# HJakeCunningham/ASVGP

Hardware: AMD Instinct MI355X
Metric: Mpoints/s per ELBO+grad step, N=10M 1D Matern-3/2 M=2048 (higher is better)
Workload: dtype f64

## Files before the change

asvgp_amd/_lib.py:

```python
import ctypes
import os

import torch

HERE = os.path.dirname(os.path.abspath(__file__))
LIB_PATH = os.path.join(HERE, "libasvgp_hip.so")

_c = ctypes
_P, _I, _L, _D, _Z = _c.c_void_p, _c.c_int, _c.c_int64, _c.c_double, _c.c_size_t

SIGNATURES = {
    "asvgp_version": (_I, []),
    "asvgp_last_error_string": (_c.c_char_p, []),
    "asvgp_status_name": (_c.c_char_p, [_I]),
    "asvgp_phi_workspace_bytes": (_Z, [_L, _I, _L]),
    "asvgp_create": (_I, [_c.POINTER(_P)]),
    "asvgp_destroy": (_I, [_P]),
    "asvgp_phi_accumulate_1d": (_I, [_P, _P, _P, _L, _L, _P, _L, _D, _I, _L, _P, _P, _Z, _P]),
    "asvgp_phi_weighted_workspace_bytes": (_Z, [_L, _I, _L]),
    "asvgp_phi_accumulate_1d_weighted": (_I, [_P, _P, _P, _P, _L, _L, _P, _L, _D, _I, _L, _P, _P, _P, _Z, _P]),
    "asvgp_set_weight_sums": (_I, [_P, _D, _D, _D]),
    "asvgp_phi_accumulate_kron2d_weighted": (_I, [_P, _P, _P, _L, _P, _L, _D, _L, _P, _L, _D, _L, _I, _P, _P, _P]),
    "asvgp_phi_accumulate_kron2d_sorted_weighted": (_I, [_P, _P, _P, _L, _P, _P, _L, _D, _L, _P, _L, _D, _L, _I, _P, _P, _P]),
    "asvgp_set_phi_algorithm": (_I, [_P, _I]),
    "asvgp_phi_last_algorithm": (_I, [_P]),
    "asvgp_set_phi_input_order": (_I, [_P, _I]),
    "asvgp_phi_last_input_order": (_I, [_P]),
    "asvgp_stream_probe": (_I, [_P, _P, _L, _P, _P]),
    "asvgp_debug_reload_env": (_I, []),
    "asvgp_set_deferred_forward_pass": (_I, [_P, _I]),
    "asvgp_prior_publish": (_I, [_P]),
    "asvgp_host_mantissa_bits": (_I, []),
    "asvgp_prior_interior_kuu_host": (_I, [_P, _I, _L, _I, _P, _P, _c.POINTER(_L), _c.POINTER(_L), _P]),
    "asvgp_result_mirror": (_I, [_P, _I, _c.POINTER(_P)]),
    "asvgp_result_mirror_read": (_I, [_P, _c.c_uint64, _P, _D]),
    "asvgp_elbo_grad_ahead_1d": (_I, [_P, _P, _P, _I, _L, _L, _I, _L, _P, _P, _P, _Z, _P]),
    "asvgp_elbo_publish_theta": (_I, [_P, _D, _D, _D]),
    "asvgp_elbo_grad_host_1d": (_I, [_P, _P, _P, _I, _D, _D, _D, _L, _L, _I, _L, _P, _P, _P, _Z, _P, _P, _D]),
    "asvgp_result_mirror_pending": (_c.c_uint64, [_P]),
    "asvgp_set_phi_workgroups": (_I, [_P, _I]),
    "asvgp_set_phi_deferred_reduce": (_I, [_P, _I]),
    "asvgp_phi_reduce_1d": (_I, [_P, _P]),
    "asvgp_phi_index_1d": (_I, [_P, _L, _P, _L, _D, _P, _P]),
    "asvgp_phi_evaluate_1d": (_I, [_P, _L, _P, _L, _D, _I, _I, _P, _P, _P]),
    "asvgp_matern_coeffs": (_I, [_I, _D, _D, _c.POINTER(_D), _c.POINTER(_D), _c.POINTER(_I)]),
    "asvgp_kuu_assemble": (_I, [_P, _I, _c.POINTER(_D), _c.POINTER(_D), _L, _I, _P, _P, _P]),
    "asvgp_cholesky_band": (_I, [_P, _P, _L, _I, _P, _P]),
    "asvgp_inverse_from_cholesky_band": (_I, [_P, _P, _L, _I, _P]),
    "asvgp_solve_triang_mat": (_I, [_P, _P, _P, _L, _I, _L, _I, _P]),
    "asvgp_product_band_band": (_I, [_P, _P, _P, _L, _I, _I, _I, _I, _I, _I, _P]),
    "asvgp_transpose_band": (_I, [_P, _P, _L, _I, _I, _P]),
    "asvgp_symmetrise_band": (_I, [_P, _P, _L, _I, _P]),
    "asvgp_unpack_banded_matrix_to_dense": (_I, [_P, _P, _L, _I, _I, _P]),
    "asvgp_pack_dense_matrix_to_banded": (_I, [_P, _P, _L, _I, _I, _P]),
    "asvgp_band_trace_sym": (_I, [_P, _P, _L, _I, _P, _P]),
    "asvgp_cholesky_band_vjp": (_I, [_P, _P, _P, _P, _L, _I, _P]),
    "asvgp_inverse_from_cholesky_band_vjp": (_I, [_P, _P, _P, _P, _P, _L, _I, _P]),
    "asvgp_band_outer_product": (_I, [_P, _P, _L, _L, _I, _D, _P, _P]),
    "asvgp_elbo_workspace_bytes": (_Z, [_L, _I, _L]),
    "asvgp_set_band_algorithm": (_I, [_P, _I]),
    "asvgp_prior_plan_1d": (_I, [_P, _P, _I, _L, _I, _c.POINTER(_I)]),
    "asvgp_prior_table_doubles": (_Z, [_P, _I, _L, _I]),
    "asvgp_prior_forward_host": (_I, [_P, _I, _L, _I, _P, _P, _P, _Z, _P]),
    "asvgp_set_prior_forward": (_I, [_P, _I]),
# ... 144 lines not shown
            self._mirror = None
            return None
        self._mirror = np.ctypeslib.as_array(ctypes.cast(ptr, ctypes.POINTER(_D)), shape=(16,))
        return self._mirror

    def set_deferred_forward_pass(self, on):
        check(self._lib.asvgp_set_deferred_forward_pass(self.ptr, int(on)), "set_deferred_forward_pass")

    def publish_forward(self):
        self._lib.asvgp_prior_publish(self.ptr)

    def result_mirror_pending(self):
        return int(self._lib.asvgp_result_mirror_pending(self.ptr))

    def set_phi_workgroups(self, n):
        check(self._lib.asvgp_set_phi_workgroups(self.ptr, int(n)), "set_phi_workgroups")

    deferred = False

    def set_phi_deferred_reduce(self, on):
        check(self._lib.asvgp_set_phi_deferred_reduce(self.ptr, int(on)), "set_phi_deferred_reduce")
        self.deferred = bool(on)

    def chain_sync(self, on):
        check(self._lib.asvgp_elbo_chain_sync(self.ptr, int(on)), "elbo_chain_sync")

    def prior_plan(self, static_stack_host, n_terms, M, k):
        ok = _I(0)
        ptr = None if static_stack_host is None else static_stack_host.ctypes.data
        check(self._lib.asvgp_prior_plan_1d(self.ptr, ptr, int(n_terms), int(M), int(k), ctypes.byref(ok)), "prior_plan_1d")
        return bool(ok.value)

    def close(self):
        if getattr(self, "ptr", None) is not None and self.ptr:
            try:
                self._lib.asvgp_destroy(self.ptr)
            except Exception:
                pass
            self.ptr = None
            self._mirror = None

    def __del__(self):
        self.close()


def set_default_algorithms(band=None, phi=None, prior_forward=None, phi_order=None):
# ... 45 lines not shown
```

asvgp_amd/csrc/handle.hip:

```cpp
#include <sched.h>
#include <stdlib.h>
#include <string.h>
#include <time.h>

#include <condition_variable>
#include <mutex>
#include <thread>
#include <vector>

#include "handle.hpp"

namespace asvgp {

static DebugEnv g_dbg;
static std::once_flag g_dbg_once;
static void debug_env_load() {
  g_dbg.no_assembly = getenv("ASVGP_DEBUG_NO_ASSEMBLY") ? 1 : 0;
  g_dbg.chain_stamps = getenv("ASVGP_CHAIN_STAMPS") ? 1 : 0;
  g_dbg.spin_limit = getenv("ASVGP_SPIN_LIMIT") ? atol(getenv("ASVGP_SPIN_LIMIT")) : (1L << 25);
  g_dbg.host_times = getenv("ASVGP_HOST_TIMES") ? 1 : 0;
  g_dbg.plan_first = getenv("ASVGP_PLAN_FIRST") ? 1 : 0;
  g_dbg.bcr_stamps = getenv("ASVGP_BCR_STAMPS") ? atoi(getenv("ASVGP_BCR_STAMPS")) : 0;
  g_dbg.no_split = getenv("ASVGP_NO_SPLIT") ? atoi(getenv("ASVGP_NO_SPLIT")) : 0;
}
const DebugEnv& debug_env() {
  std::call_once(g_dbg_once, debug_env_load);
  return g_dbg;
}

static Handle* g_default = nullptr;
static std::mutex g_default_mu;

Handle* as_handle(asvgp_handle_t h) {
  if (h) return reinterpret_cast<Handle*>(h);
  std::lock_guard<std::mutex> lk(g_default_mu);
  if (!g_default) {
    g_default = new Handle;
    (void)hipGetDevice(&g_default->device);
  }
  return g_default;
}

static void handle_quiesce(Handle* h) {
  if (h->ahead.valid) (void)elbo_publish_theta(h, 1.0, 1.0, 1.0, true);
  handle_publish_forward(h);
  bool need_sync = false;
// ... 164 lines not shown
  return ASVGP_OK;
}

extern "C" int asvgp_create(asvgp_handle_t* out) {
  if (!out) { set_error("asvgp_create: bad argument"); return ASVGP_ERR_BAD_ARG; }
  Handle* h = new Handle;
  if (hipGetDevice(&h->device) != hipSuccess) { delete h; set_error("asvgp_create: no HIP device"); return ASVGP_ERR_HIP; }
  *out = reinterpret_cast<asvgp_handle_t>(h);
  return ASVGP_OK;
}

extern "C" int asvgp_destroy(asvgp_handle_t handle) {
  if (!handle) return ASVGP_OK;
  Handle* h = reinterpret_cast<Handle*>(handle);
  if (h->magic != 0x41535647u) { set_error("asvgp_destroy: not a handle"); return ASVGP_ERR_BAD_ARG; }
  worker_stop(h);
  plan_release(h);
  if (h->mirror_host) (void)hipHostFree(h->mirror_host);
  if (h->evK) (void)hipEventDestroy(h->evK);
  if (h->evP) (void)hipEventDestroy(h->evP);
  if (h->prof_made)
    for (int i = 0; i < PROF_RING; ++i) { (void)hipEventDestroy(h->prof_ev[i][0]); (void)hipEventDestroy(h->prof_ev[i][1]); }
  if (h->order_dev) { (void)hipFree(h->order_dev); h->order_dev = nullptr; }
  if (h->box_host) { (void)hipHostFree(h->box_host); h->box_host = nullptr; h->box_dev = nullptr; }
  h->magic = 0;
  delete h;
  return ASVGP_OK;
}

extern "C" int asvgp_set_phi_algorithm(asvgp_handle_t handle, int algo) {
  if (algo != 0 && algo != 1 && algo != 3 && algo != 5 && algo != 6) {
    set_error("set_phi_algorithm: 0 auto (6 where it applies, else 5, else 3), 1 fp64 LDS-atomic band scatter, 3 fixed-point band scatter, 5 fixed-point centred-moment scatter, 6 tile sort + register moments");
    return ASVGP_ERR_BAD_ARG;
  }
  as_handle(handle)->phi_algo = algo;
  return ASVGP_OK;
}

extern "C" int asvgp_set_phi_input_order(asvgp_handle_t handle, int order) {
  if (order < 0 || order > 2) { set_error("set_phi_input_order: 0 probe once per (x, N), 1 unsorted, 2 time series"); return ASVGP_ERR_BAD_ARG; }
  Handle* h = as_handle(handle);
  h->phi_order = order;
  h->n_order_seen = 0;
  return ASVGP_OK;
}

// ... 2 lines not shown
extern "C" int asvgp_set_phi_workgroups(asvgp_handle_t handle, int n) {
  if (n < 0 || n > 256) { set_error("set_phi_workgroups: 0 (default, one per CU) .. 256"); return ASVGP_ERR_BAD_ARG; }
  as_handle(handle)->phi_blocks = n;
  return ASVGP_OK;
}

extern "C" int asvgp_set_weight_sums(asvgp_handle_t handle, double n_pos, double sum_w, double sum_log_w) {
  Handle* h = as_handle(handle);
  if (n_pos < 0.0) { h->w_set = false; h->w_npos = h->w_sum = h->w_sumlog = 0.0; return ASVGP_OK; }
  if (!(n_pos == n_pos) || n_pos != (double)(long long)n_pos || n_pos > 9.0e15 || !(sum_w >= 0.0) || !(sum_w < 1e300) || !(fabs(sum_log_w) < 1e300)) {
    set_error("set_weight_sums: n_pos must be a whole number of rows (negative: unweighted), sum_w >= 0 and sum_log_w finite");
    return ASVGP_ERR_BAD_ARG;
  }
  h->w_set = true; h->w_npos = n_pos; h->w_sum = sum_w; h->w_sumlog = sum_log_w;
  return ASVGP_OK;
}

extern "C" int asvgp_set_phi_deferred_reduce(asvgp_handle_t handle, int on) {
  Handle* h = as_handle(handle);
  h->phi_defer = on != 0;
  if (!h->phi_defer) h->pend.valid = false;
  return ASVGP_OK;
}

extern "C" int asvgp_set_band_algorithm(asvgp_handle_t handle, int algo) {
  if (algo < 0 || algo > 4) {
    set_error("set_band_algorithm: 0 auto, 1 sequential sweeps, 2 block cyclic reduction on the GPU, 3 block cyclic reduction with the planned (host, long double) prior forward pass, 4 the planned chains on the matrix cores");
    return ASVGP_ERR_BAD_ARG;
  }
  as_handle(handle)->band_algo = algo;
  return ASVGP_OK;
}

extern "C" int asvgp_set_deferred_forward_pass(asvgp_handle_t handle, int on) {
  Handle* h = as_handle(handle);
  if (on < 0 || on > 2) { set_error("set_deferred_forward_pass: 0 inline, 1 the caller publishes (asvgp_prior_publish), 2 the handle's worker thread"); return ASVGP_ERR_BAD_ARG; }
  handle_publish_forward(h);
  if (on != 2) worker_stop(h);
  h->defer_forward = on == 1;
  h->fwd_worker = on == 2;
  return ASVGP_OK;
}

extern "C" int asvgp_prior_publish(asvgp_handle_t handle) {
  handle_publish_forward(as_handle(handle));
  return ASVGP_OK;
// ... 143 lines not shown
```

asvgp_amd/csrc/handle.hpp:

```cpp
#pragma once
#include "asvgp_common.hpp"
#include "prior_plan.hpp"

namespace asvgp {

constexpr int PROF_RING = 1024;
constexpr int TAB_SLOTS = 16;

struct Handle {
  unsigned magic = 0x41535647u;
  int device = 0;
  int phi_algo = 0, phi_blocks = 0;
  int phi_last = 0;
  bool phi_defer = false;
  struct PendingReduce { const double* partials; int G, M, K; double* stats; bool valid; const int* ranges; } pend = {nullptr, 0, 0, 0, nullptr, false, nullptr};
  int band_algo = 0;
  bool sync_on = false;
  hipEvent_t evK = nullptr, evP = nullptr;
  bool prof_on = false, prof_made = false;
  int prof_every = 1;
  long prof_calls = 0, prof_n = 0;
  hipEvent_t prof_ev[PROF_RING][2];
  PriorPlan* plan = nullptr;
  int* node_rec_dev = nullptr;
// ... 12 lines not shown
  void* worker_park = nullptr;
  int wstate = 0;
  struct PendingForward { bool valid; double coef[ASVGP_MAX_KUU_TERMS], dcoef[ASVGP_MAX_KUU_TERMS]; double* tab; int slot; unsigned long long seq; } fwd = {false, {0}, {0}, nullptr, 0, 0};
  bool prior_forward_gpu = false;
  int* dd_img_i = nullptr;
  int dd_n_img = 0;
  double* dd_img_d = nullptr;
  double* dd_tab = nullptr;
  hipStream_t dd_stream = nullptr;
  unsigned long long* dd_ready = nullptr;
  double* mirror_host = nullptr;
  double* mirror_dev = nullptr;
  unsigned long long mirror_seq = 0;
  unsigned long long mirror_pending = 0;
  struct MeshSeen { const double* ptr; long n; int regular; double step, first, last; };
  MeshSeen mesh_seen[8];
  int n_mesh_seen = 0;
  int phi_order = 0;
  struct OrderSeen { const double* ptr; long n; int series; };
  OrderSeen order_seen[8];
  int n_order_seen = 0;
  int* order_dev = nullptr;
  int phi_last_series = 0;
  bool ahead_req = false;
  void* box_host = nullptr;
  void* box_dev = nullptr;
  struct PendingAhead { bool valid; int slot; unsigned long long seq; double* tab; int kind; double N, Nw, cw; } ahead = {false, 0, 0, nullptr, 0, 0.0, 0.0, 0.0};
  bool w_set = false;
  double w_npos = 0.0, w_sum = 0.0, w_sumlog = 0.0;
};
constexpr size_t BOX_BYTES = 4096;

struct DebugEnv { int no_assembly; int chain_stamps; long spin_limit; int host_times; int plan_first; int bcr_stamps; int no_split; };
const DebugEnv& debug_env();

Handle* as_handle(asvgp_handle_t h);

bool handle_mesh_is_linspace(Handle* h, const double* mesh_dev, long n_mesh, hipStream_t st, double* step_out, double* first_out, double* last_out);

int handle_flush_phi_reduce(Handle* h, const double* stats, hipStream_t st);

void handle_publish_forward(Handle* h);
void handle_post_forward(Handle* h);

int handle_prior_dd_prepare(Handle* h);
void handle_prior_dd_release(Handle* h);
int handle_prior_dd_forward(Handle* h, const double* coef, const double* dcoef, int slot, hipStream_t st, double** tab_out, unsigned long long* stamps = nullptr,
                            unsigned long long seq = 0, const unsigned long long** ready_out = nullptr);

int elbo_publish_theta(Handle* h, double v, double l, double s, bool withdraw);

double* handle_table_acquire(Handle* h, unsigned long long* seq_out, int* slot_out);

}
```

asvgp_amd/csrc/phi_pass.hip:

```cpp
#include <stdlib.h>

#include "handle.hpp"

namespace asvgp {

constexpr int PHI_THREADS = 1024;
constexpr int PHI_CH = 32;
constexpr int PHI_MAX_BLOCKS = 256;
constexpr size_t PHI_LDS_BUDGET = 160 * 1024 - 512;

template <int K> struct FxTab {
  int g[K + 1];
  constexpr FxTab() : g{} {
    double cf[K + 1][K + 1] = {};
    for (int i = 0; i <= K; ++i)
      for (int p = 0; p <= K; ++p) cf[i][p] = piece_coef<K, 0>(i, p);
    for (int d = 0; d <= K; ++d) {
      double mx = 0.0;
      for (int i = 0; i + d <= K; ++i)
        for (int q = 0; q <= 32; ++q) {
          const double t = q / 32.0;
          double a = cf[i][K], b = cf[i + d][K];
          for (int p = K - 1; p >= 0; --p) { a = a * t + cf[i][p]; b = b * t + cf[i + d][p]; }
          if (a * b > mx) mx = a * b;
// ... 658 lines not shown
  if (lane == 0 && good) atomicAdd(count, 1);
}

static bool handle_phi_is_series(Handle* h, const double* x, long N, double m0, double inv_delta, long n_mesh, hipStream_t st) {
  if (h->phi_order == 1) return false;
  if (h->phi_order == 2) return true;
  for (int i = 0; i < h->n_order_seen; ++i)
    if (h->order_seen[i].ptr == x && h->order_seen[i].n == N) return h->order_seen[i].series != 0;
  int series = 0;
  const int nprobe = 512;
  if (N >= 128L * nprobe) {
    if (!h->order_dev && hipMalloc(&h->order_dev, sizeof(int)) != hipSuccess) h->order_dev = nullptr;
    int cnt = 0;
    if (h->order_dev && hipMemsetAsync(h->order_dev, 0, sizeof(int), st) == hipSuccess) {
      hipLaunchKernelGGL(phi_order_probe_kernel, dim3(nprobe), dim3(64), 0, st, x, N, N / nprobe, nprobe, m0, inv_delta, (int)n_mesh, h->order_dev);
      if (hipMemcpyAsync(&cnt, h->order_dev, sizeof(int), hipMemcpyDeviceToHost, st) == hipSuccess && hipStreamSynchronize(st) == hipSuccess)
        series = cnt * 10 >= nprobe * 9 ? 1 : 0;
    }
  }
  if (h->n_order_seen < 8) h->order_seen[h->n_order_seen++] = Handle::OrderSeen{x, N, series};
  return series != 0;
}

template <int K, int TP, int TS>
static int launch_phi_sort_as(Handle* h, const double* x, const double* y, long N, const double* mesh, long n_mesh, double delta,
                              long M, double* stats, double* ws, hipStream_t st, double step, double m0, double m_last, double margin) {
  size_t lds_bytes = ps_lds_bytes<K, TP, TS>();
  if (ps_epilogue_bytes<K>() > lds_bytes) lds_bytes = ps_epilogue_bytes<K>();
  if (lds_bytes > 160 * 1024) return 1;
  long nblk = (N + TP * PS_THREADS - 1) / (TP * PS_THREADS);
  const long gmax = (h->phi_blocks > 0 && h->phi_blocks < PHI_MAX_BLOCKS) ? h->phi_blocks : PHI_MAX_BLOCKS;
  const int G = (int)(nblk < 1 ? 1 : (nblk > gmax ? gmax : nblk));
  long ppb = (N + G - 1) / G;
  ppb = TS ? ((ppb + 127) & ~127L) : ((ppb + 1) & ~1L);
  if (ppb > 0x3fffffffL) return 1;
  PsArgs a;
  a.x = x; a.y = y; a.N = N; a.mesh_g = mesh; a.n_mesh = (int)n_mesh; a.inv_delta = 1.0 / delta; a.M = (int)M;
  a.m0 = m0; a.m_last = m_last; a.step = step; a.smax_fast = 0.5 - margin;
  a.partials = ws; a.ppb = ppb; a.zero_ptr = stats; a.zero_n = (K + 2) * M + 1; a.stamps = nullptr; a.stamps_wave = 0;
  a.ranges = reinterpret_cast<int*>(ws + (size_t)PHI_MAX_BLOCKS * ((size_t)(K + 2) * M + 1));
  auto kern = phi_sort_kernel<K, TP, 0, 1, TS>;
  hipError_t e = hipFuncSetAttribute(reinterpret_cast<const void*>(kern), hipFuncAttributeMaxDynamicSharedMemorySize, (int)lds_bytes);
  if (e != hipSuccess) { set_error("hipFuncSetAttribute(%zu B LDS): %s", lds_bytes, hipGetErrorString(e)); return ASVGP_ERR_LDS_CAPACITY; }
  const bool prof = h->prof_on && h->prof_n < PROF_RING && (h->prof_calls++ % h->prof_every == 0);
  if (prof) (void)hipEventRecord(h->prof_ev[h->prof_n][0], st);
  hipLaunchKernelGGL(kern, dim3((unsigned)G), dim3(PS_THREADS), lds_bytes, st, a);
  if (prof) { (void)hipEventRecord(h->prof_ev[h->prof_n][1], st); ++h->prof_n; }
  h->phi_last_series = TS;
  const int E1 = (int)((K + 2) * M + 1);
  const int gsplit = G >= 64 ? 16 : (G >= 8 ? 4 : 1);
  if (h->phi_defer) {
    h->pend = Handle::PendingReduce{a.partials, G, (int)M, K, stats, true, a.ranges};
    return check_launch("phi_accumulate_1d (tile sort, reduce deferred)");
  }
  hipLaunchKernelGGL(phi_reduce_kernel, dim3((E1 + 255) / 256, gsplit), dim3(256), 0, st, a.partials, G, (int)M, K, 0, M, 1L, 0, 1, stats, (const int*)a.ranges);
  return check_launch("phi_accumulate_1d (tile sort)");
}

template <int K>
static int launch_phi_sort(Handle* h, const double* x, const double* y, long N, long D, const double* mesh, long n_mesh, double delta,
                           long M, double* stats, double* ws, hipStream_t st) {
  if (D != 1 || N < 2 || M > PS_NCELL || ((reinterpret_cast<uintptr_t>(x) | reinterpret_cast<uintptr_t>(y)) & 15) != 0) return 1;
  double step = 0.0, m0 = 0.0, m_last = 0.0;
  if (!handle_mesh_is_linspace(h, mesh, n_mesh, st, &step, &m0, &m_last)) return 1;
  const double amax = fabs(m0) > fabs(m_last) ? fabs(m0) : fabs(m_last);
  const double margin = 16.0 * 2.220446049250313e-16 * amax / delta + 1e-12;
  if (!(margin < 0.125)) return 1;
  constexpr int TP = ps_tile_points<K>();
  constexpr int TPS = TP < 4 ? TP : 4;
  if (handle_phi_is_series(h, x, N, m0, 1.0 / delta, n_mesh, st)) {
    const int rc = launch_phi_sort_as<K, TPS, 1>(h, x, y, N, mesh, n_mesh, delta, M, stats, ws, st, step, m0, m_last, margin);
    if (rc != 1) return rc;
  }
  return launch_phi_sort_as<K, TP, 0>(h, x, y, N, mesh, n_mesh, delta, M, stats, ws, st, step, m0, m_last, margin);
}

template <int K>
static int launch_phi(Handle* h, const double* x, const double* y, long N, long D, const double* mesh, long n_mesh,
                      double delta, long M, double* stats, double* partials, hipStream_t st) {
  { const int rcf = handle_flush_phi_reduce(h, nullptr, st); if (rcf) return rcf; }
  const int ncells = (int)n_mesh - 1;
  if (h->phi_algo == 0 || h->phi_algo == 6) {
    const int rc = launch_phi_sort<K>(h, x, y, N, D, mesh, n_mesh, delta, M, stats, partials, st);
    if (rc != 1) { h->phi_last = 6; return rc; }
    if (h->phi_algo == 6) { set_error("phi algorithm 6 (tile sort) needs D == 1, N >= 2, M <= 2048, 16-byte aligned x / y and a mesh that is an exact linspace"); return ASVGP_ERR_UNSUPPORTED; }
  }
  if (h->phi_algo == 0 || h->phi_algo == 5) {
    const int rc = launch_phi_moments<K>(h, x, y, N, D, mesh, n_mesh, delta, M, stats, partials, st);
    if (rc != 1) { h->phi_last = 5; return rc; }
    if (h->phi_algo == 5) { set_error("phi algorithm 5 (centred moments) needs D == 1, 16-byte aligned x / y and M small enough for the LDS split"); return ASVGP_ERR_UNSUPPORTED; }
  }
  const bool fx = (h->phi_algo != 1);
  h->phi_last = fx ? 3 : 1;
  int maxc = phi_max_cols(K, n_mesh, fx);
  if (maxc < 2 * K + 2) {
    set_error("phi_accumulate_1d: mesh table (%ld knots) leaves no LDS for the band", n_mesh);
    return ASVGP_ERR_LDS_CAPACITY;
  }
  int cells_per_chunk = (M <= maxc) ? ncells : (maxc - K);
  long nblk = (N + 2 * PHI_THREADS - 1) / (2 * PHI_THREADS);
  const long gmax = (h->phi_blocks > 0 && h->phi_blocks < PHI_MAX_BLOCKS) ? h->phi_blocks : PHI_MAX_BLOCKS;
  int G = (int)(nblk < 1 ? 1 : (nblk > gmax ? gmax : nblk));
  long ppb = (N + G - 1) / G;
// ... 277 lines not shown
```

asvgp_amd/csrc/phi_sort.hpp:

```cpp
#pragma once

namespace asvgp {

constexpr int PS_THREADS = 1024;
constexpr int PS_NCELL = 2 * PS_THREADS;
constexpr int PS_HEAVY = 48;
constexpr int PS_HROUND = 16;
constexpr int PS_HLIST = 8192 / (PS_HEAVY + 1) + 1;

struct PsArgs {
  const double* x; const double* y; long N;
  const double* mesh_g; int n_mesh; double inv_delta; int M;
  double m0, m_last;
  double step;
  double smax_fast;
  double* partials;
  long ppb;
  double* zero_ptr; long zero_n;
  unsigned long long* stamps;
  int stamps_wave;
  int* ranges;
};

template <int K> constexpr int ps_tile_points() { return K <= 3 ? 8 : (K == 4 ? 6 : (K == 5 ? 4 : 2)); }
#ifndef PS_GW
#define PS_GW 4
#endif
constexpr int PS_TS_SLOTS = 256;
template <int K> constexpr size_t ps_ts_bytes() { return (size_t)PS_TS_SLOTS * (3 * K + 2) * 8 + (size_t)2 * PS_TS_SLOTS * 4; }
template <int K, int TP, int TS = 0> constexpr size_t ps_lds_bytes() {
  return (size_t)(TP * PS_THREADS + 1) * 16 + (size_t)3 * PS_NCELL * 4 + 64 * 4 + 64 * 8 +
         (size_t)PS_HROUND * (3 * K + 1) * 8 + (size_t)PS_HLIST * 12 + (TS ? ps_ts_bytes<K>() : 0);
}
template <int K> constexpr size_t ps_epilogue_bytes() {
  int all = (K + 1) * (K + 2) / 2, lo = (K + 1) + K, hi = all - lo;
  int planes = K <= 4 ? all : (lo > hi ? lo : hi);
  if (planes < 2 * (K + 1)) planes = 2 * (K + 1);
  return (size_t)planes * (PS_THREADS + K) * 8;
}

__device__ __forceinline__ void ps_lds_barrier() { asm volatile("s_waitcnt lgkmcnt(0)\n\ts_barrier" ::: "memory"); }

template <int CTRL, int ROW_MASK>
__device__ __forceinline__ unsigned ps_dpp_add_u32(unsigned v) {
  return v + (unsigned)__builtin_amdgcn_update_dpp(0, (int)v, CTRL, ROW_MASK, 0xf, true);
// ... 86 lines not shown
  for (int q = 0; q <= K; ++q) T2[q] = 0.0;
  for (unsigned sl = (unsigned)first; sl < nsl; sl += (unsigned)stride) {
    const unsigned j = sl * 64 + lane;
    if (j < hn) {
      const double2 pt = buf[ho + j];
      ps_acc<K>(pt.x, pt.y, S2, T2);
    }
  }
  if constexpr (NS <= 8) {
    int idx;
    const double t = ps_reduce_scatter8<NS>(S2, lane, idx);
    if (lane < 8 && idx < NS) lds_add(slot + idx, t);
  } else {
#pragma unroll
    for (int q = 0; q < NS; ++q) { const double t = wave_sum_dpp(S2[q]); if (lane == 0) lds_add(slot + q, t); }
  }
  __builtin_amdgcn_sched_barrier(0);
  {
    int idx;
    const double t = ps_reduce_scatter8<K + 1>(T2, lane, idx);
    if (lane < 8 && idx <= K) lds_add(slot + NS + idx, t);
  }
  __builtin_amdgcn_sched_barrier(0);
}

template <int K, int TP, int ABL = 0, int PF = 0, int TS = 0>
__global__ __launch_bounds__(PS_THREADS) void phi_sort_kernel(PsArgs a) {
  extern __shared__ double lds[];
  static_assert(TP % 2 == 0 && TP * PS_THREADS <= 8192, "tile: rank field is 13 bits");
  constexpr int T = TP * PS_THREADS;
  constexpr int NS = 2 * K;
  double2* buf = reinterpret_cast<double2*>(lds);
  unsigned* cnt = reinterpret_cast<unsigned*>(buf + T + 1);
  unsigned* off = cnt + 2 * PS_NCELL;
  unsigned* wtot = off + PS_NCELL;
  double* scratch = reinterpret_cast<double*>(wtot + 64);
  constexpr int NSTAT = 3 * K + 1;
  double* hacc = scratch + 64;
  unsigned* hlist = reinterpret_cast<unsigned*>(hacc + PS_HROUND * NSTAT);
  unsigned* nheavy_p = wtot + 32;
  constexpr int TSW = NSTAT + 1;
  double* tstab = reinterpret_cast<double*>(hlist + 3 * PS_HLIST);
  int* tskey = reinterpret_cast<int*>(tstab + PS_TS_SLOTS * TSW);
  int* tslist = tskey + PS_TS_SLOTS;
  unsigned* ts_ctl = wtot + 40;
  if (a.zero_ptr) for (long e = (long)blockIdx.x * blockDim.x + threadIdx.x; e < a.zero_n; e += (long)gridDim.x * blockDim.x) a.zero_ptr[e] = 0.0;
  const int tid0 = threadIdx.x;
  int tid = tid0, lane = tid0 & 63, wv = tid0 >> 6;
  const int n_mesh = a.n_mesh, ncells = n_mesh - 1, M = a.M;
  const double* __restrict__ mesh = a.mesh_g;
  const double inv_delta = a.inv_delta, step = a.step, smax_fast = a.smax_fast;
  const double m0 = a.m0, m_last = a.m_last;
  {
    uint4* z = reinterpret_cast<uint4*>(cnt);
    z[tid] = make_uint4(0u, 0u, 0u, 0u);
    if (tid == 0) { buf[T] = make_double2(0.0, 0.0); ts_ctl[0] = 0; ts_ctl[1] = 0; }
    if constexpr (TS == 1) {
      if (tid < PS_TS_SLOTS) tskey[tid] = -1;
      for (int e = tid; e < PS_TS_SLOTS * TSW; e += PS_THREADS) tstab[e] = 0.0;
    }
  }
  unsigned nbad = 0;
  auto knot = [&](int i) __attribute__((always_inline)) -> double { return (i == n_mesh - 1) ? m_last : mq_linspace_knot(i, step, m0); };
  auto cell_slow = [&](double x, double& s_out, bool& ok) __attribute__((always_inline)) -> int {
    int i = mq_guess(x, m0, inv_delta, n_mesh);
    const double k0 = knot(i);
    const bool down = !(k0 < x) && i > 0;
    const bool up = !down && i < n_mesh - 2 && knot(i + 1) < x;
// ... 437 lines not shown
#pragma unroll
        for (int p = 0; p < NS; ++p) SB[p] += sl[p];
#pragma unroll
        for (int p = 0; p <= K; ++p) TB[p] += sl[NS + p];
        n0B += (unsigned)sl[NSTAT];
      }
    }
  }
  double tot = block_sum(yy, scratch);
  const double badf = block_sum((double)nbad, scratch + 32);
  __syncthreads();
  double* out = a.partials + (size_t)blockIdx.x * ((size_t)(K + 2) * M + 1);
  int col_lo = 0, col_hi = M - 1;
  if (a.ranges) {
    const unsigned mn = n0A ? (unsigned)tid : (n0B ? (unsigned)(tid + PS_THREADS) : 0x7fffffu);
    const unsigned mx = n0B ? (unsigned)(tid + PS_THREADS) + 1u : (n0A ? (unsigned)tid + 1u : 0u);
    const unsigned wmn = ps_wave_min_u32(mn), wmx = ps_wave_max_u32(mx);
    if (lane == 0) { wtot[wv] = wmn; wtot[16 + wv] = wmx; }
    __syncthreads();
    const unsigned bmn = ps_wave_min_u32(wtot[lane & 15]), bmx = ps_wave_max_u32(wtot[16 + (lane & 15)]);
    col_lo = bmx ? (int)bmn : 1;
    col_hi = bmx ? (int)bmx - 1 + K : 0;
    if (col_hi > M - 1) col_hi = M - 1;
    if (tid == 0) { a.ranges[2 * blockIdx.x] = col_lo; a.ranges[2 * blockIdx.x + 1] = col_hi; }
    __syncthreads();
  }
  if constexpr (ABL == 5) {
    double keep = (double)(n0A + n0B);
#pragma unroll
    for (int p = 0; p < NS; ++p) keep += SA[p] + SB[p];
#pragma unroll
    for (int p = 0; p <= K; ++p) keep += TA[p] + TB[p];
    out[tid] = keep;
  } else if constexpr (ABL == 0 || ABL == 9) {
    constexpr int IW = PS_THREADS + K;
    double* img = lds;
    auto q_planes = [&](const double (&S)[NS], unsigned n0, int slot, int d0, int d1) __attribute__((always_inline)) {
      const double s0v = (double)n0;
      int pid = 0;
      if (!__any(n0 != 0u)) {
#pragma unroll
        for (int d = d0; d < d1; ++d)
#pragma unroll
          for (int i = 0; i + d <= K; ++i) img[(pid++) * IW + slot] = 0.0;
        return;
      }
#pragma unroll
      for (int d = d0; d < d1; ++d) {
#pragma unroll
        for (int i = 0; i + d <= K; ++i) {
          const int j = i + d, mi = K - j, mj = K - i;
          if (mi < i) continue;
          double e = MomCoef<K>::tab.pair[i][j][0] * s0v, o = 0.0;
#pragma unroll
          for (int p = 2; p <= NS; p += 2) e = fma(MomCoef<K>::tab.pair[i][j][p], S[p - 1], e);
          if (mi != i) {
#pragma unroll
            for (int p = 1; p <= NS; p += 2) o = fma(MomCoef<K>::tab.pair[i][j][p], S[p - 1], o);
            img[(pid + mi) * IW + slot] = e - o;
// ... 24 lines not shown
#pragma unroll
      for (int rnd = 0; rnd < (DSPLIT <= K ? 2 : 1); ++rnd) {
        const int d0 = rnd == 0 ? 0 : DSPLIT, d1 = rnd == 0 ? DSPLIT : K + 1;
        if (half == 0) q_planes(SA, n0A, K + tid, d0, d1); else q_planes(SB, n0B, K + tid, d0, d1);
        if (tid >= PS_THREADS - K) {
          const int hs = tid - (PS_THREADS - K);
          if (half == 0) {
            int np = 0;
#pragma unroll
            for (int d = d0; d < d1; ++d) np += K + 1 - d;
            for (int pl = 0; pl < np; ++pl) img[pl * IW + hs] = 0.0;
          } else {
            q_planes(SA, n0A, hs, d0, d1);
          }
        }
        ps_lds_barrier();
        if (j < M && j >= col_lo && j <= col_hi) {
          int pid = 0;
#pragma unroll
          for (int d = d0; d < d1; ++d) {
            double v = 0.0;
#pragma unroll
            for (int jj = d; jj <= K; ++jj) v += img[(pid + jj - d) * IW + tid + jj];
            __builtin_nontemporal_store((j + d < M) ? v : 0.0, out + (size_t)d * M + j);
            pid += K + 1 - d;
          }
        }
        ps_lds_barrier();
      }
    }
    r_planes(TA, K + tid, 0);
    r_planes(TB, K + tid, K + 1);
    if (tid >= PS_THREADS - K) {
      const int hs = tid - (PS_THREADS - K);
#pragma unroll
      for (int i = 0; i <= K; ++i) img[i * IW + hs] = 0.0;
      r_planes(TA, hs, K + 1);
    }
    ps_lds_barrier();
#pragma unroll
    for (int half = 0; half < 2; ++half) {
      const int j = half * PS_THREADS + tid;
      if (j < M && j >= col_lo && j <= col_hi) {
        double r = 0.0;
#pragma unroll
        for (int i = 0; i <= K; ++i) r += img[(half * (K + 1) + i) * IW + tid + i];
        __builtin_nontemporal_store(r, out + (size_t)(K + 1) * M + j);
      }
    }
    if (tid == 0) out[(size_t)(K + 2) * M] = (badf > 0.0) ? __builtin_nan("") : tot;
  } else {
    if (tid == 0) out[0] = tot + badf;
  }
  stamp(4);
  if constexpr (ABL == 9) {
    if (tid == (int)(a.stamps_wave * 64) && a.stamps)
      for (int i = 0; i < 8; ++i) a.stamps[(size_t)blockIdx.x * 8 + i] = ph[i];
  }
}

}
```

asvgp_amd/gpr.py:

```python
import ctypes
import math
import time

import numpy as np
import torch
import torch.distributed as dist

from . import kernels, utils
from . import kernels as kernels_mod
from ._lib import AsvgpError, Handle, check, f64c, get_lib, require_cuda, stream_ptr
from .banded import NotPositiveDefiniteError
from .dist import allreduce_stats
from .inducing_features import SplineFeatures1D


def _to_device(a, device):
    t = torch.as_tensor(a)
    return f64c(t.to(device))


def _require_inside(col, a, b, strict, what):
    if col.numel() == 0:
        return
    lo, hi = torch.aminmax(col)
# ... 1500 lines not shown
        for i, bs in enumerate(bases):
            _require_inside(self.X[:, i], bs.a, bs.b, True, "GPR_additive dimension %d" % i)
        lib = get_lib()
        ms = [bs.m for bs in bases]
        self.offsets = [0]
        for m in ms:
            self.offsets.append(self.offsets[-1] + m)
        self.Mtot = self.offsets[-1]
        self._diag_off, self._cross_off, o = [], {}, 0
        for m in ms:
            self._diag_off.append(o)
            o += (k + 2) * m + 1
        for i in range(self.d):
            for j in range(i + 1, self.d):
                self._cross_off[(i, j)] = o
                o += ms[i] * ms[j]
        self._stats = torch.empty(o, dtype=torch.float64, device=dev)
        self._cols = [self.X[:, i].contiguous() for i in range(self.d)]
        wsb = max([lib.asvgp_phi_workspace_bytes(m, k, 1) for m in ms] +
                  [lib.asvgp_phi_cross_workspace_bytes(ms[i], ms[j]) for (i, j) in self._cross_off] + [8])
        self._ws = torch.empty(wsb // 8 + 1, dtype=torch.float64, device=dev)
        self._wsb = wsb
        self._h = Handle()
        self._setup_dist(process_group, distributed)
        self._phi_pass_local()
        self.num_data = allreduce_stats(self._stats, self.n, process_group) if self._distributed else self.n
        self.tr_yTy = self._stats[self._diag_off[0] + (k + 2) * ms[0]]
        self._info = torch.zeros(1, dtype=torch.int32, device=dev)
        self._dense = None
        self._post_cov = None
        self._post_alpha = None

    def _phi_pass_local(self):
        lib, k = get_lib(), self.bandwidth
        for i, bs in enumerate(self.bases):
            out = self._stats[self._diag_off[i]:]
            check(lib.asvgp_phi_accumulate_1d(self._h.ptr, self._cols[i].data_ptr(), self.y.data_ptr(), self.n, 1, bs.mesh.data_ptr(),
                                              bs.mesh.shape[0], bs.delta_np, k, bs.m, out.data_ptr(), self._ws.data_ptr(),
                                              self._wsb, stream_ptr()), "phi_accumulate_1d")
        check(lib.asvgp_phi_reduce_1d(self._h.ptr, stream_ptr()), "phi_reduce_1d")
        for (i, j), o in self._cross_off.items():
            bi, bj = self.bases[i], self.bases[j]
            check(lib.asvgp_phi_cross_2d(self._cols[i].data_ptr(), self._cols[j].data_ptr(), self.n, bi.mesh.data_ptr(),
                                         bi.mesh.shape[0], bi.delta_np, bi.m, bj.mesh.data_ptr(), bj.mesh.shape[0],
                                         bj.delta_np, bj.m, k, self._stats[o:].data_ptr(), self._ws.data_ptr(), self._wsb,
                                         stream_ptr()), "phi_cross_2d")
# ... 284 lines not shown
```

include/asvgp_hip.h:

```cpp
#ifndef ASVGP_HIP_H
#define ASVGP_HIP_H

#include <stddef.h>
#include <stdint.h>

#ifdef __cplusplus
extern "C" {
#endif

typedef void* asvgp_stream_t;
typedef struct asvgp_handle_s* asvgp_handle_t;

typedef enum {
  ASVGP_OK = 0,
  ASVGP_ERR_BAD_ARG = -1,
  ASVGP_ERR_UNSUPPORTED = -2,
  ASVGP_ERR_LDS_CAPACITY = -3,
  ASVGP_ERR_WORKSPACE = -4,
  ASVGP_ERR_HIP = -5
} asvgp_status;

enum { ASVGP_MATERN12 = 0, ASVGP_MATERN32 = 1, ASVGP_MATERN52 = 2 };
enum { ASVGP_MAX_ORDER = 6, ASVGP_MAX_BANDWIDTH = 8, ASVGP_MAX_KUU_TERMS = 9 };

// ... 13 lines not shown
int asvgp_prior_interior_kuu_host(const double* static_bands_host, int n_terms, int64_t M, int k, const double* coef_host,
                                  double* kuu_diag8, int64_t* lo, int64_t* hi, double* bnd256);
int asvgp_host_mantissa_bits(void);
int asvgp_debug_reload_env(void);
int asvgp_set_deferred_forward_pass(asvgp_handle_t handle, int on);
int asvgp_prior_publish(asvgp_handle_t handle);
int asvgp_result_mirror(asvgp_handle_t handle, int enable, const double** host_ptr);
uint64_t asvgp_result_mirror_pending(asvgp_handle_t handle);
int asvgp_result_mirror_read(asvgp_handle_t handle, uint64_t token, double* result10, double timeout_seconds);
int asvgp_elbo_grad_ahead_1d(asvgp_handle_t handle, const double* stats, const double* static_bands, int kind, int64_t N, int64_t M, int k,
                             int64_t D, double* out, int* info, void* workspace, size_t workspace_bytes, asvgp_stream_t stream);
int asvgp_elbo_publish_theta(asvgp_handle_t handle, double variance, double lengthscale, double noise_variance);
int asvgp_elbo_grad_host_1d(asvgp_handle_t handle, const double* stats, const double* static_bands, int kind, double variance,
                            double lengthscale, double noise_variance, int64_t N, int64_t M, int k, int64_t D,
                            double* out, int* info, void* workspace, size_t workspace_bytes, asvgp_stream_t stream,
                            double* result10, double timeout_seconds);
int asvgp_phi_last_algorithm(asvgp_handle_t handle);
int asvgp_set_phi_input_order(asvgp_handle_t handle, int order);
int asvgp_phi_last_input_order(asvgp_handle_t handle);
int asvgp_stream_probe(const double* x, const double* y, int64_t N, double* sink, asvgp_stream_t stream);
int asvgp_set_phi_workgroups(asvgp_handle_t handle, int n);
int asvgp_set_phi_deferred_reduce(asvgp_handle_t handle, int on);
int asvgp_phi_reduce_1d(asvgp_handle_t handle, asvgp_stream_t stream);

size_t asvgp_phi_weighted_workspace_bytes(int64_t M, int order, int64_t D);
int asvgp_phi_accumulate_1d_weighted(asvgp_handle_t handle, const double* x, const double* y, const double* w, int64_t N, int64_t D,
                                     const double* mesh, int64_t n_mesh, double delta, int order, int64_t M, double* stats,
                                     double* wstats, void* workspace, size_t workspace_bytes, asvgp_stream_t stream);
int asvgp_set_weight_sums(asvgp_handle_t handle, double n_pos, double sum_w, double sum_log_w);

int asvgp_phi_index_1d(const double* x, int64_t N, const double* mesh, int64_t n_mesh, double delta,
                       int64_t* idx, asvgp_stream_t stream);

int asvgp_phi_evaluate_1d(const double* x, int64_t N, const double* mesh, int64_t n_mesh, double delta,
                          int order, int deriv, int64_t* rows, double* data, asvgp_stream_t stream);

int asvgp_matern_coeffs(int kind, double variance, double lengthscale, double* coef_host, double* dcoef_dl_host,
                        int* n_terms_host);
int asvgp_kuu_assemble(const double* static_bands, int n_terms, const double* coef_host,
                       const double* dcoef_dl_host, int64_t M, int k, double* Kuu, double* dKuu_dl,
                       asvgp_stream_t stream);

int asvgp_cholesky_band(const double* K, double* L, int64_t M, int k, int* info, asvgp_stream_t stream);
int asvgp_inverse_from_cholesky_band(const double* L, double* S, int64_t M, int k, asvgp_stream_t stream);
int asvgp_solve_triang_mat(const double* L, const double* B, double* X, int64_t M, int k, int64_t D,
                           int transpose_left, asvgp_stream_t stream);
// ... 175 lines not shown
```

Before: 134,200.

## Fuse cross-workgroup partial reduction into phi sort kernel tail

```diff
diff --git a/asvgp_amd/_lib.py b/asvgp_amd/_lib.py
--- a/asvgp_amd/_lib.py
+++ b/asvgp_amd/_lib.py
@@ -40,6 +40,8 @@
     "asvgp_result_mirror_pending": (_c.c_uint64, [_P]),
     "asvgp_set_phi_workgroups": (_I, [_P, _I]),
     "asvgp_set_phi_deferred_reduce": (_I, [_P, _I]),
+    "asvgp_set_phi_inkernel_reduce": (_I, [_P, _I]),
+    "asvgp_phi_last_inkernel_reduce": (_I, [_P]),
     "asvgp_phi_reduce_1d": (_I, [_P, _P]),
     "asvgp_phi_index_1d": (_I, [_P, _L, _P, _L, _D, _P, _P]),
     "asvgp_phi_evaluate_1d": (_I, [_P, _L, _P, _L, _D, _I, _I, _P, _P, _P]),
@@ -230,6 +232,12 @@
         check(self._lib.asvgp_set_phi_deferred_reduce(self.ptr, int(on)), "set_phi_deferred_reduce")
         self.deferred = bool(on)
 
+    def set_phi_inkernel_reduce(self, mode):
+        check(self._lib.asvgp_set_phi_inkernel_reduce(self.ptr, int(mode)), "set_phi_inkernel_reduce")
+
+    def phi_last_inkernel_reduce(self):
+        return int(self._lib.asvgp_phi_last_inkernel_reduce(self.ptr))
+
     def chain_sync(self, on):
         check(self._lib.asvgp_elbo_chain_sync(self.ptr, int(on)), "elbo_chain_sync")
 
diff --git a/asvgp_amd/csrc/handle.hip b/asvgp_amd/csrc/handle.hip
--- a/asvgp_amd/csrc/handle.hip
+++ b/asvgp_amd/csrc/handle.hip
@@ -22,6 +22,8 @@
   g_dbg.plan_first = getenv("ASVGP_PLAN_FIRST") ? 1 : 0;
   g_dbg.bcr_stamps = getenv("ASVGP_BCR_STAMPS") ? atoi(getenv("ASVGP_BCR_STAMPS")) : 0;
   g_dbg.no_split = getenv("ASVGP_NO_SPLIT") ? atoi(getenv("ASVGP_NO_SPLIT")) : 0;
+  g_dbg.phi_inkernel = getenv("ASVGP_PHI_INKERNEL") ? atoi(getenv("ASVGP_PHI_INKERNEL")) : 1;
+  if (g_dbg.phi_inkernel < 0 || g_dbg.phi_inkernel > 2) g_dbg.phi_inkernel = 1;
 }
 const DebugEnv& debug_env() {
   std::call_once(g_dbg_once, debug_env_load);
@@ -232,6 +234,7 @@
   if (h->prof_made)
     for (int i = 0; i < PROF_RING; ++i) { (void)hipEventDestroy(h->prof_ev[i][0]); (void)hipEventDestroy(h->prof_ev[i][1]); }
   if (h->order_dev) { (void)hipFree(h->order_dev); h->order_dev = nullptr; }
+  if (h->phi_sync_dev) { (void)hipFree(h->phi_sync_dev); h->phi_sync_dev = nullptr; }
   if (h->box_host) { (void)hipHostFree(h->box_host); h->box_host = nullptr; h->box_dev = nullptr; }
   h->magic = 0;
   delete h;
@@ -280,6 +283,14 @@
   if (!h->phi_defer) h->pend.valid = false;
   return ASVGP_OK;
 }
+
+extern "C" int asvgp_set_phi_inkernel_reduce(asvgp_handle_t handle, int mode) {
+  if (mode < -1 || mode > 2) { set_error("set_phi_inkernel_reduce: -1 as ASVGP_PHI_INKERNEL says (default on), 0 off, 1 on, 2 on and no workgroup waits"); return ASVGP_ERR_BAD_ARG; }
+  as_handle(handle)->phi_inkernel = mode;
+  return ASVGP_OK;
+}
+
+extern "C" int asvgp_phi_last_inkernel_reduce(asvgp_handle_t handle) { return as_handle(handle)->phi_last_inkernel; }
 
 extern "C" int asvgp_set_band_algorithm(asvgp_handle_t handle, int algo) {
   if (algo < 0 || algo > 4) {
diff --git a/asvgp_amd/csrc/handle.hpp b/asvgp_amd/csrc/handle.hpp
--- a/asvgp_amd/csrc/handle.hpp
+++ b/asvgp_amd/csrc/handle.hpp
@@ -58,6 +58,11 @@
   int n_order_seen = 0;
   int* order_dev = nullptr;
   int phi_last_series = 0;
+  int phi_inkernel = -1;
+  int phi_last_inkernel = 0;
+  unsigned long long* phi_sync_dev = nullptr;
+  unsigned long long phi_sync_seq = 0;
+  int cu_count = 0;
   bool ahead_req = false;
   void* box_host = nullptr;
   void* box_dev = nullptr;
@@ -67,7 +72,7 @@
 };
 constexpr size_t BOX_BYTES = 4096;
 
-struct DebugEnv { int no_assembly; int chain_stamps; long spin_limit; int host_times; int plan_first; int bcr_stamps; int no_split; };
+struct DebugEnv { int no_assembly; int chain_stamps; long spin_limit; int host_times; int plan_first; int bcr_stamps; int no_split; int phi_inkernel; };
 const DebugEnv& debug_env();
 
 Handle* as_handle(asvgp_handle_t h);
diff --git a/asvgp_amd/csrc/phi_pass.hip b/asvgp_amd/csrc/phi_pass.hip
--- a/asvgp_amd/csrc/phi_pass.hip
+++ b/asvgp_amd/csrc/phi_pass.hip
@@ -704,6 +704,18 @@
   return series != 0;
 }
 
+static int handle_phi_inkernel_mode(Handle* h, int G) {
+  const int mode = h->phi_inkernel >= 0 ? h->phi_inkernel : debug_env().phi_inkernel;
+  if (!mode) return 0;
+  if (!h->cu_count && hipDeviceGetAttribute(&h->cu_count, hipDeviceAttributeMultiprocessorCount, h->device) != hipSuccess) h->cu_count = 0;
+  if (G > h->cu_count) return 0;
+  if (!h->phi_sync_dev) {
+    if (hipMalloc(&h->phi_sync_dev, PS_SYNC_WORDS * sizeof(unsigned long long)) != hipSuccess) { (void)hipGetLastError(); h->phi_sync_dev = nullptr; return 0; }
+    if (hipMemset(h->phi_sync_dev, 0, PS_SYNC_WORDS * sizeof(unsigned long long)) != hipSuccess) { (void)hipGetLastError(); (void)hipFree(h->phi_sync_dev); h->phi_sync_dev = nullptr; return 0; }
+  }
+  return mode;
+}
+
 template <int K, int TP, int TS>
 static int launch_phi_sort_as(Handle* h, const double* x, const double* y, long N, const double* mesh, long n_mesh, double delta,
                               long M, double* stats, double* ws, hipStream_t st, double step, double m0, double m_last, double margin) {
@@ -721,6 +733,11 @@
   a.m0 = m0; a.m_last = m_last; a.step = step; a.smax_fast = 0.5 - margin;
   a.partials = ws; a.ppb = ppb; a.zero_ptr = stats; a.zero_n = (K + 2) * M + 1; a.stamps = nullptr; a.stamps_wave = 0;
   a.ranges = reinterpret_cast<int*>(ws + (size_t)PHI_MAX_BLOCKS * ((size_t)(K + 2) * M + 1));
+  const int red_mode = handle_phi_inkernel_mode(h, G);
+  if (red_mode) {
+    a.red_mode = red_mode; a.sync = h->phi_sync_dev; a.tag = (++h->phi_sync_seq) << 16; a.spin_limit = debug_env().spin_limit; a.stats = stats;
+    a.zero_ptr = nullptr; a.zero_n = 0;
+  }
   auto kern = phi_sort_kernel<K, TP, 0, 1, TS>;
   hipError_t e = hipFuncSetAttribute(reinterpret_cast<const void*>(kern), hipFuncAttributeMaxDynamicSharedMemorySize, (int)lds_bytes);
   if (e != hipSuccess) { set_error("hipFuncSetAttribute(%zu B LDS): %s", lds_bytes, hipGetErrorString(e)); return ASVGP_ERR_LDS_CAPACITY; }
@@ -729,6 +746,8 @@
   hipLaunchKernelGGL(kern, dim3((unsigned)G), dim3(PS_THREADS), lds_bytes, st, a);
   if (prof) { (void)hipEventRecord(h->prof_ev[h->prof_n][1], st); ++h->prof_n; }
   h->phi_last_series = TS;
+  h->phi_last_inkernel = red_mode;
+  if (red_mode) return check_launch("phi_accumulate_1d (tile sort, reduce in the kernel)");
   const int E1 = (int)((K + 2) * M + 1);
   const int gsplit = G >= 64 ? 16 : (G >= 8 ? 4 : 1);
   if (h->phi_defer) {
@@ -761,6 +780,7 @@
 static int launch_phi(Handle* h, const double* x, const double* y, long N, long D, const double* mesh, long n_mesh,
                       double delta, long M, double* stats, double* partials, hipStream_t st) {
   { const int rcf = handle_flush_phi_reduce(h, nullptr, st); if (rcf) return rcf; }
+  h->phi_last_inkernel = 0;
   const int ncells = (int)n_mesh - 1;
   if (h->phi_algo == 0 || h->phi_algo == 6) {
     const int rc = launch_phi_sort<K>(h, x, y, N, D, mesh, n_mesh, delta, M, stats, partials, st);
diff --git a/asvgp_amd/csrc/phi_sort.hpp b/asvgp_amd/csrc/phi_sort.hpp
--- a/asvgp_amd/csrc/phi_sort.hpp
+++ b/asvgp_amd/csrc/phi_sort.hpp
@@ -20,7 +20,14 @@
   unsigned long long* stamps;
   int stamps_wave;
   int* ranges;
+  int red_mode = 0;
+  unsigned long long* sync = nullptr;
+  unsigned long long tag = 0;
+  long spin_limit = 0;
+  double* stats = nullptr;
 };
+constexpr int PS_SYNC_CENSUS = 0, PS_SYNC_TICKET = 16, PS_SYNC_CLAIM = 32;
+constexpr int PS_SYNC_WORDS = PS_SYNC_CLAIM + 256;
 
 template <int K> constexpr int ps_tile_points() { return K <= 3 ? 8 : (K == 4 ? 6 : (K == 5 ? 4 : 2)); }
 #ifndef PS_GW
@@ -153,6 +160,127 @@
     if (lane < 8 && idx <= K) lds_add(slot + NS + idx, t);
   }
   __builtin_amdgcn_sched_barrier(0);
+}
+
+__device__ __forceinline__ unsigned long long ps_count_in(unsigned long long* w, unsigned long long tag) {
+  (void)__hip_atomic_fetch_max(w, tag, __ATOMIC_RELAXED, __HIP_MEMORY_SCOPE_AGENT);
+  return __hip_atomic_fetch_add(w, 1ull, __ATOMIC_RELAXED, __HIP_MEMORY_SCOPE_AGENT);
+}
+
+struct PsTailArgs { int red_mode, M; unsigned long long* sync; unsigned long long tag; long spin_limit; double* stats; const double* partials; const int* ranges; };
+__device__ __forceinline__ PsTailArgs ps_tail_args() {
+  typedef const PsArgs __attribute__((address_space(4))) * ka_t;
+  ka_t ka = (ka_t)__builtin_amdgcn_kernarg_segment_ptr();
+  asm volatile("" : "+s"(ka));
+  PsTailArgs t;
+  t.red_mode = ka->red_mode; t.M = ka->M; t.sync = ka->sync; t.tag = ka->tag; t.spin_limit = ka->spin_limit; t.stats = ka->stats;
+  t.partials = ka->partials; t.ranges = ka->ranges;
+  return t;
+}
+
+template <int K>
+__device__ __forceinline__ void ps_tail_reduce(double* lds, int tid) {
+  typedef unsigned long long u64;
+  const PsTailArgs a = ps_tail_args();
+  const int G = (int)gridDim.x, b = (int)blockIdx.x, M = a.M;
+  const int E1 = (K + 2) * M + 1;
+  u64* const ticket = a.sync + PS_SYNC_TICKET;
+  u64* const claim = a.sync + PS_SYNC_CLAIM;
+  const u64 WILL = a.tag | 1ull, TAKEN = a.tag | 2ull;
+  int* ctl = reinterpret_cast<int*>(lds);
+  int* list = ctl + 16;
+  int* rng = list + 256;
+  double* comb = lds + 512;
+  bool will = false;
+  if (tid == 0 && a.red_mode == 1 && G > 1 &&
+      __hip_atomic_load(a.sync + PS_SYNC_CENSUS, __ATOMIC_RELAXED, __HIP_MEMORY_SCOPE_AGENT) == a.tag + (u64)G) {
+    __hip_atomic_store(claim + b, WILL, __ATOMIC_RELAXED, __HIP_MEMORY_SCOPE_AGENT);
+    will = true;
+  }
+  asm volatile("s_waitcnt vmcnt(0)" ::: "memory");
+  __syncthreads();
+  if (tid == 0) {
+    const u64 drawn = ps_count_in(ticket, a.tag) - a.tag;
+    int role = 0;
+    if (drawn == (u64)(G - 1)) {
+      role = 2;
+    } else if (will) {
+      bool all = false;
+      for (long spins = 0; spins < a.spin_limit; ++spins) {
+        if (__hip_atomic_load(ticket, __ATOMIC_RELAXED, __HIP_MEMORY_SCOPE_AGENT) == a.tag + (u64)G) { all = true; break; }
+        __builtin_amdgcn_s_sleep(16);
+      }
+      if (all && __hip_atomic_exchange(claim + b, TAKEN, __ATOMIC_RELAXED, __HIP_MEMORY_SCOPE_AGENT) != TAKEN) role = 1;
+    }
+    if (role) {
+      __builtin_amdgcn_fence(__ATOMIC_ACQUIRE, "agent");
+      asm volatile("s_waitcnt vmcnt(0)" ::: "memory");
+    }
+    ctl[0] = role; ctl[1] = 0;
+  }
+  __syncthreads();
+  const int role = ctl[0];
+  if (role == 0) return;
+  if (a.ranges) {
+    if (tid < 2 * G) rng[tid] = __hip_atomic_load(a.ranges + tid, __ATOMIC_RELAXED, __HIP_MEMORY_SCOPE_AGENT);
+    __syncthreads();
+  }
+  const int pps = ((E1 + 7) / 8 + G - 1) / G;
+  const int per = (G + 15) / 16;
+  const int q = tid >> 6, c = tid & 63;
+  const int g0 = q * per, g1 = (g0 + per < G) ? g0 + per : G;
+  const bool ranged = a.ranges != nullptr;
+  auto reduce_slice = [&](int s) __attribute__((always_inline)) {
+    const int lo = s * pps * 8;
+    const int hi = (lo + pps * 8 < E1) ? lo + pps * 8 : E1;
+    for (int c0 = lo; c0 < hi; c0 += 64) {
+      const int e = c0 + c;
+      double acc = 0.0;
+      if (e < hi) {
+        const int colr = e < (K + 2) * M ? e % M : -1;
+        const double* src = a.partials + e;
+        for (int g = g0; g < g1; g += 16) {
+          double v[16];
+#pragma unroll
+          for (int u = 0; u < 16; ++u) {
+            const int gg = g + u;
+            bool ok = gg < g1;
+            if (ok && ranged && colr >= 0) ok = colr >= rng[2 * gg] && colr <= rng[2 * gg + 1];
+            v[u] = ok ? __hip_atomic_load(src + (size_t)gg * E1, __ATOMIC_RELAXED, __HIP_MEMORY_SCOPE_AGENT) : 0.0;
+          }
+#pragma unroll
+          for (int u = 0; u < 16; ++u) acc += v[u];
+        }
+      }
+      comb[q * 64 + c] = acc;
+      __syncthreads();
+      if (tid < 64 && e < hi) {
+        double t = comb[tid];
+#pragma unroll
+        for (int w = 1; w < 16; ++w) t += comb[w * 64 + tid];
+        a.stats[e] = t;
+      }
+      __syncthreads();
+    }
+  };
+  if (role == 1) { reduce_slice(b); return; }
+  for (int pass = 0; pass < 2; ++pass) {
+    if (tid < G) {
+      bool go = true;
+      if (pass == 0 && tid != b) {
+        const u64 v = __hip_atomic_load(claim + tid, __ATOMIC_RELAXED, __HIP_MEMORY_SCOPE_AGENT);
+        go = v != WILL && v != TAKEN;
+      }
+      if (go && __hip_atomic_exchange(claim + tid, TAKEN, __ATOMIC_RELAXED, __HIP_MEMORY_SCOPE_AGENT) != TAKEN)
+        list[atomicAdd(&ctl[1], 1)] = tid;
+    }
+    __syncthreads();
+    const int n = ctl[1];
+    for (int i = 0; i < n; ++i) reduce_slice(list[i]);
+    __syncthreads();
+    if (tid == 0) ctl[1] = 0;
+    __syncthreads();
+  }
 }
 
 template <int K, int TP, int ABL = 0, int PF = 0, int TS = 0>
@@ -175,6 +303,7 @@
   int* tskey = reinterpret_cast<int*>(tstab + PS_TS_SLOTS * TSW);
   int* tslist = tskey + PS_TS_SLOTS;
   unsigned* ts_ctl = wtot + 40;
+  if (a.red_mode && threadIdx.x == 0) ps_count_in(a.sync + PS_SYNC_CENSUS, a.tag);
   if (a.zero_ptr) for (long e = (long)blockIdx.x * blockDim.x + threadIdx.x; e < a.zero_n; e += (long)gridDim.x * blockDim.x) a.zero_ptr[e] = 0.0;
   const int tid0 = threadIdx.x;
   int tid = tid0, lane = tid0 & 63, wv = tid0 >> 6;
@@ -658,7 +787,12 @@
     col_lo = bmx ? (int)bmn : 1;
     col_hi = bmx ? (int)bmx - 1 + K : 0;
     if (col_hi > M - 1) col_hi = M - 1;
-    if (tid == 0) { a.ranges[2 * blockIdx.x] = col_lo; a.ranges[2 * blockIdx.x + 1] = col_hi; }
+    if (tid == 0) {
+      if (ps_tail_args().red_mode) {
+        __hip_atomic_store(a.ranges + 2 * blockIdx.x, col_lo, __ATOMIC_RELAXED, __HIP_MEMORY_SCOPE_AGENT);
+        __hip_atomic_store(a.ranges + 2 * blockIdx.x + 1, col_hi, __ATOMIC_RELAXED, __HIP_MEMORY_SCOPE_AGENT);
+      } else { a.ranges[2 * blockIdx.x] = col_lo; a.ranges[2 * blockIdx.x + 1] = col_hi; }
+    }
     __syncthreads();
   }
   if constexpr (ABL == 5) {
@@ -671,6 +805,10 @@
   } else if constexpr (ABL == 0 || ABL == 9) {
     constexpr int IW = PS_THREADS + K;
     double* img = lds;
+    const bool wt = ps_tail_args().red_mode != 0;
+    auto put = [&](double v, double* p) __attribute__((always_inline)) {
+      if (wt) __hip_atomic_store(p, v, __ATOMIC_RELAXED, __HIP_MEMORY_SCOPE_AGENT); else __builtin_nontemporal_store(v, p);
+    };
     auto q_planes = [&](const double (&S)[NS], unsigned n0, int slot, int d0, int d1) __attribute__((always_inline)) {
       const double s0v = (double)n0;
       int pid = 0;
@@ -741,7 +879,7 @@
             double v = 0.0;
 #pragma unroll
             for (int jj = d; jj <= K; ++jj) v += img[(pid + jj - d) * IW + tid + jj];
-            __builtin_nontemporal_store((j + d < M) ? v : 0.0, out + (size_t)d * M + j);
+            put((j + d < M) ? v : 0.0, out + (size_t)d * M + j);
             pid += K + 1 - d;
           }
         }
@@ -764,10 +902,11 @@
         double r = 0.0;
 #pragma unroll
         for (int i = 0; i <= K; ++i) r += img[(half * (K + 1) + i) * IW + tid + i];
-        __builtin_nontemporal_store(r, out + (size_t)(K + 1) * M + j);
-      }
-    }
-    if (tid == 0) out[(size_t)(K + 2) * M] = (badf > 0.0) ? __builtin_nan("") : tot;
+        put(r, out + (size_t)(K + 1) * M + j);
+      }
+    }
+    if (tid == 0) put((badf > 0.0) ? __builtin_nan("") : tot, out + (size_t)(K + 2) * M);
+    if (wt) ps_tail_reduce<K>(lds, tid);
   } else {
     if (tid == 0) out[0] = tot + badf;
   }
diff --git a/asvgp_amd/gpr.py b/asvgp_amd/gpr.py
--- a/asvgp_amd/gpr.py
+++ b/asvgp_amd/gpr.py
@@ -1546,6 +1546,7 @@
         self._ws = torch.empty(wsb // 8 + 1, dtype=torch.float64, device=dev)
         self._wsb = wsb
         self._h = Handle()
+        self._h.set_phi_inkernel_reduce(0)
         self._setup_dist(process_group, distributed)
         self._phi_pass_local()
         self.num_data = allreduce_stats(self._stats, self.n, process_group) if self._distributed else self.n
diff --git a/include/asvgp_hip.h b/include/asvgp_hip.h
--- a/include/asvgp_hip.h
+++ b/include/asvgp_hip.h
@@ -59,6 +59,8 @@
 int asvgp_set_phi_workgroups(asvgp_handle_t handle, int n);
 int asvgp_set_phi_deferred_reduce(asvgp_handle_t handle, int on);
 int asvgp_phi_reduce_1d(asvgp_handle_t handle, asvgp_stream_t stream);
+int asvgp_set_phi_inkernel_reduce(asvgp_handle_t handle, int mode);
+int asvgp_phi_last_inkernel_reduce(asvgp_handle_t handle);
 
 size_t asvgp_phi_weighted_workspace_bytes(int64_t M, int order, int64_t D);
 int asvgp_phi_accumulate_1d_weighted(asvgp_handle_t handle, const double* x, const double* y, const double* w, int64_t N, int64_t D,
```

Result: slower. 116,500 (-13.2%).
